# akashsengupta1997/indirect_learning_pose-shape

Measured on AMD Instinct MI355X. Metric: meshes/sec fwd+bwd (SMPL->48x48 31-part seg), higher is better.
Workload: dtype f32; 1 GPU; full decoder fwd+bwd (batch_smpl + projection + compute_mask + projects_to_seg), BASELINE configs[2]; meshes_per_gpu=128, global_batch=128, img_wh=48, vertex_sampling=1, verts=6890, params_per_mesh=86, launch=graph, steps_per_graph_launch=10, concurrent_chunks=1

## Files before the change

### include/smplraster.h

```cpp
#ifndef SMPLRASTER_H
#define SMPLRASTER_H

#include <stddef.h>
#include <stdint.h>

#ifdef __cplusplus
extern "C" {
#endif

#define SMPLR_ABI_VERSION 7
#define SMPLR_NJ 24
#define SMPLR_KPAD 220
#define SMPLR_CHUNK 8

#define SMPLR_EINVAL (-1)
#define SMPLR_EUNSUPPORTED (-2)

int smplr_abi_version(void);
const char *smplr_last_error(void);
int smplr_debug_device_ordinal(int fake_ordinal);
int smplr_debug_lds_attr_sets(void);
const char *smplr_build_id(void);


// ... 87 lines not shown
                           int16_t *arg, float *kernel_ms, void *stream);

int smplr_seg_raster_plan(int B, int W, int P, int K, int32_t *info, int32_t *tile_records);

int smplr_seg_bwd_nsplit(int B, int W);
size_t smplr_seg_bwd_workspace(int B, int W);
int smplr_seg_bwd(const float *dseg, const int16_t *arg, const float *rec,
                  int B, int VP, int W, int P, int K, float *dproj, void *workspace, int deterministic,
                  void *stream);

int smplr_seg_raster_ex(int B, int W, int P, int K, const void *workspace, const float *rec,
                        const int32_t *labels, const float *class_w, float gamma, float *seg, int16_t *arg,
                        float *loss, float *stats, float *vmax, void *stream);
int smplr_skin_vis_seg_fwd_ex(const float *v_posed, const float *lbs_top4, const float *A, const float *cam,
                              int x_stride, int B, int V, int W, int grid_wh, int ref_compat,
                              const int32_t *part_pos, const int32_t *part_off, int P, int K, void *workspace,
                              const int32_t *labels, const float *class_w, float gamma, float *verts, float *proj,
                              float *mask, float *seg, int16_t *arg, float *rec, int16_t *vslot, float *loss,
                              float *stats, float *vmax, void *stream);
int smplr_seg_loss_bwd(const float *dloss, const float *stats, const int16_t *arg, const float *rec, int B, int VP,
                       int W, int P, int K, float *dproj, void *workspace, int deterministic, void *stream);

int smplr_seg_confusion(const float *scores, const int32_t *pred, const int32_t *labels, long long npix, int C,
                        uint64_t *conf, uint8_t *pred_out, void *stream);
int smplr_seg_raster_ex_conf(int B, int W, int P, int K, const void *workspace, const float *rec,
                             const int32_t *labels, const float *class_w, float gamma, float *seg, int16_t *arg,
                             float *loss, float *stats, float *vmax, uint64_t *conf, void *stream);
int smplr_skin_vis_seg_fwd_ex_conf(const float *v_posed, const float *lbs_top4, const float *A, const float *cam,
                                   int x_stride, int B, int V, int W, int grid_wh, int ref_compat,
                                   const int32_t *part_pos, const int32_t *part_off, int P, int K, void *workspace,
                                   const int32_t *labels, const float *class_w, float gamma, float *verts, float *proj,
                                   float *mask, float *seg, int16_t *arg, float *rec, int16_t *vslot, float *loss,
                                   float *stats, float *vmax, uint64_t *conf, void *stream);

#define SMPLR_MESH_ORTHO 0
#define SMPLR_MESH_PERSPECTIVE 1
#define SMPLR_MESH_LAMBERT 0
#define SMPLR_MESH_VERTEX_COLOR 1
size_t smplr_mesh_vbuf_bytes(int B, int V);
int smplr_mesh_vertex(const float *verts, const float *cam, const float *trans, int B, int V, int mode, float scale,
                      int H, int W, float znear, float zfar, int shading, const int32_t *faces, int F,
                      const int32_t *vf_off, const int32_t *vf_face, int nnz, const float *light, int nlights,
                      const float *vcol, long long vcol_bstride, void *vbuf, void *stream);
int smplr_mesh_raster(const void *vbuf, const int32_t *faces, const uint8_t *face_part, int B, int V, int F, int H,
                      int W, int mode, const float *bg, int32_t *face, float *depth, uint8_t *part, uint8_t *alpha,
                      float *rgb, void *stream);

#define SMPLR_WARP_IMAGE_NEAREST 0
#define SMPLR_WARP_IMAGE_BILINEAR 1
#define SMPLR_WARP_LABEL 2
#define SMPLR_WARP_LABEL_BINARY 3
int smplr_affine_warp(const uint8_t *pool, int N, int Hs, int Ws, int C, const float *mat, const void *index,
                      int index_i64, int B, int H, int W, int mode, float rescale, void *out, void *stream);

#define SMPLR_RESIZE_IMAGE_BILINEAR 0
#define SMPLR_RESIZE_IMAGE_NEAREST 1
#define SMPLR_RESIZE_LABEL 2
#define SMPLR_RESIZE_LABEL_BINARY 3
#define SMPLR_RESIZE_PAD 1
#define SMPLR_RESIZE_SWAP_RB 2
#define SMPLR_RESIZE_QUANTIZE 4
#define SMPLR_RESIZE_PIL 8
int smplr_resize_pad(const uint8_t *data, long long data_bytes, const long long *desc, int N, int C, const void *index,
                     int index_i64, int B, int H, int W, int mode, int flags, float rescale, void *out, void *stream);

#define SMPLR_PE_NONE 0
// ... 120 lines not shown
```

### indirect_learning_pose-shape_amd/_lib.py

```python
from __future__ import annotations

import ctypes
import os
from ctypes import c_char_p, c_float, c_int, c_longlong, c_size_t, c_void_p

import torch

_HERE = os.path.dirname(os.path.abspath(__file__))
LIB_OVERRIDE = os.environ.get("SMPLR_LIB_PATH") or None
LIB_PATH = os.path.abspath(LIB_OVERRIDE) if LIB_OVERRIDE else os.path.join(_HERE, "libsmplraster_hip.so")

KPAD = 220
CHUNK = 8
ABI_VERSION = 7

P = c_void_p
I = c_int

SIGNATURES = {
    "smplr_abi_version": (c_int, []),
    "smplr_last_error": (c_char_p, []),
    "smplr_build_id": (c_char_p, []),
    "smplr_debug_device_ordinal": (c_int, [I]),
    "smplr_debug_lds_attr_sets": (c_int, []),
# ... 11 lines not shown
    "smplr_blend3_fwd": (c_int, [P, P, P, I, I, P, P]),
    "smplr_pose_blend3_fwd": (c_int, [P, I, I, I, P, P, P, P, P, I, P, P, P, P, P, P]),
    "smplr_blend3_bwd_workspace": (c_size_t, [I, I]),
    "smplr_blend3_bwd": (c_int, [P, P, I, I, P, P, P]),
    "smplr_skin_fwd": (c_int, [P, P, P, P, P, I, I, I, I, P, P, P]),
    "smplr_skin_bwd_workspace": (c_size_t, [I, I]),
    "smplr_skin_bwd": (c_int, [P, P, P, P, P, P, P, I, I, I, I, P, P, P, P, P]),
    "smplr_smpl_bwd_workspace": (c_size_t, [I, I]),
    "smplr_smpl_bwd": (c_int, [P, P, P, P, I, P, P, I, I, I, I, I, P, P, P, P, P, P, P, P, P, P, P, P, P]),
    "smplr_project_fwd": (c_int, [P, P, I, I, I, I, P, P]),
    "smplr_project_bwd": (c_int, [P, P, P, I, I, I, I, P, P, P]),
    "smplr_visibility": (c_int, [P, I, I, I, I, P, P]),
    "smplr_seg_workspace": (c_size_t, [I, I, I, I, I]),
    "smplr_seg_slots": (c_int, [I, I]),
    "smplr_seg_fwd": (c_int, [P, P, I, I, I, P, P, I, I, P, P, P, P, P, P]),
    "smplr_vis_seg_fwd": (c_int, [P, I, I, I, I, I, P, P, I, I, P, P, P, P, P, P, P]),
    "smplr_skin_vis_seg_fits": (c_int, [I, I, I]),
    "smplr_skin_vis_seg_fwd": (c_int, [P, P, P, P, I, I, I, I, I, I, P, P, I, I, P, P, P, P, P, P, P, P, P]),
    "smplr_seg_bin": (c_int, [P, P, I, I, I, I, I, P, P, I, I, P, P, P, P]),
    "smplr_seg_raster": (c_int, [I, I, I, I, P, P, P, P, P]),
    "smplr_seg_raster_timed": (c_int, [I, I, I, I, P, P, P, P, P, P]),
    "smplr_seg_raster_plan": (c_int, [I, I, I, I, P, P]),
    "smplr_seg_bwd_nsplit": (c_int, [I, I]),
    "smplr_seg_bwd_workspace": (c_size_t, [I, I]),
    "smplr_seg_bwd": (c_int, [P, P, P, I, I, I, I, I, P, P, I, P]),
    "smplr_seg_raster_ex": (c_int, [I, I, I, I, P, P, P, P, c_float, P, P, P, P, P, P]),
    "smplr_skin_vis_seg_fwd_ex": (c_int, [P, P, P, P, I, I, I, I, I, I, P, P, I, I, P, P, P, c_float, P, P, P, P, P, P,
                                          P, P, P, P, P]),
    "smplr_seg_loss_bwd": (c_int, [P, P, P, P, I, I, I, I, I, P, P, I, P]),
    "smplr_seg_confusion": (c_int, [P, P, P, c_longlong, I, P, P, P]),
    "smplr_seg_raster_ex_conf": (c_int, [I, I, I, I, P, P, P, P, c_float, P, P, P, P, P, P, P]),
    "smplr_skin_vis_seg_fwd_ex_conf": (c_int, [P, P, P, P, I, I, I, I, I, I, P, P, I, I, P, P, P, c_float, P, P, P, P, P,
                                               P, P, P, P, P, P, P]),
    "smplr_mesh_vbuf_bytes": (c_size_t, [I, I]),
    "smplr_mesh_vertex": (c_int, [P, P, P, I, I, I, c_float, I, I, c_float, c_float, I, P, I, P, P, I, P, I, P, c_longlong,
                                  P, P]),
    "smplr_mesh_raster": (c_int, [P, P, P, I, I, I, I, I, I, P, P, P, P, P, P, P]),
    "smplr_affine_warp": (c_int, [P, I, I, I, I, P, P, I, I, I, I, I, c_float, P, P]),
    "smplr_resize_pad": (c_int, [P, c_longlong, P, I, I, P, I, I, I, I, I, I, c_float, P, P]),
    "smplr_point_errors": (c_int, [P, P, I, I, I, I, P, P, P, P, P]),
    "smplr_mesh_measures": (c_int, [P, P, P, P, c_longlong, P, I, I, I, I, P, P, P, P, P, P, P, P]),
    "smplr_mesh_measures_bwd": (c_int, [P, P, P, P, I, P, P, c_longlong, P, P, P, P, P, P, P, I, I, I, I, P, P]),
    "smplr_seg_colour": (c_int, [P, P, I, I, I, I, P, I, I, P, I, I, I, P, P]),
    "smplr_scatter_points": (c_int, [P, P, P, I, P, I, I, I, I, c_float, I, I, I, I, P, P, P]),
    "smplr_fit_step": (c_int, [P, P, P, P, P, P, P, P, P, P, P, P, P, I, P, I, c_float, P, P, I, I, I, c_float, c_float, c_float,
                               c_float, c_float, I, I, P]),
    "smplr_prior_energy": (c_int, [P, I, I, I, P, P, P, P, P, P, I, I, P, P, P, P, P]),
    "smplr_fit_step_prior": (c_int, [P, P, P, P, P, P, P, P, P, P, P, P, P, I, P, I, c_float, P, P, I, I, I, c_float, c_float,
                                     c_float, c_float, c_float, I, I, I, P, P, P, P, P, P, I, I, P, P]),
    "smplr_silh_workspace": (c_size_t, [I, I, I]),
    "smplr_silh_fwd": (c_int, [P, I, I, I, P, P, P, P]),
    "smplr_silh_fwd_hint": (c_int, [P, P, I, I, I, P, P, P, P]),
    "smplr_silh_fwd_form": (c_int, [I, I]),
    "smplr_silh_bwd": (c_int, [P, P, P, P, I, I, I, P, I, P]),
    "smplr_silh_loss_fwd": (c_int, [P, P, P, c_float, I, I, P, P, P, P]),
    "smplr_silh_fwd_loss": (c_int, [P, P, P, P, c_float, I, I, I, P, P, P, P, P, P, P]),
    "smplr_silh_loss_bwd": (c_int, [P, P, P, P, P, I, I, I, P, I, P]),
    "smplr_focal_fwd": (c_int, [P, P, P, P, c_float, c_longlong, I, P, P, P]),
    "smplr_focal_bwd": (c_int, [P, P, P, P, c_float, P, c_longlong, I, P, P]),
    "smplr_prelu_fwd": (c_int, [P, P, c_longlong, I, I, P, P]),
    "smplr_prelu_bwd_workspace": (c_size_t, [c_longlong, I, I]),
    "smplr_prelu_bwd": (c_int, [P, P, P, c_longlong, I, I, P, P, P, P]),
    "smplr_bn_workspace": (c_size_t, [c_longlong, I, I]),
    "smplr_bn_fwd": (c_int, [P, P, P, P, c_longlong, I, I, c_float, c_float, P, P, P, P, P, P, P]),
    "smplr_bn_bwd": (c_int, [P, P, P, P, P, P, P, c_longlong, I, I, P, P, P, P, P, P]),
    "smplr_bn_res_fwd": (c_int, [P, P, P, P, P, P, c_longlong, I, I, c_float, c_float, P, P, P, P, P, P, P]),
# ... 116 lines not shown
```

### indirect_learning_pose-shape_amd/csrc/raster.hip

```cpp
#include <algorithm>
#include <tuple>
#include "raster_device.h"

namespace smplr {
#ifdef SMPLR_TL
constexpr int TL_RASTER_WG = 1152;
__device__ unsigned g_tl_raster[TL_RASTER_WG * 16 * 32];
#endif

constexpr int PLN = 128;
__host__ inline int raster2_shape(int B, int W, int K) {
  const long long nl = (long long)((W + 1) / 2) * W, blocks1 = (long long)B * ((nl + PLN - 1) / PLN);
  return (W <= 48 && K >= 6000 && blocks1 <= 900) ? 2 : 1;
}
constexpr int R2_STATIC = 1;
constexpr int R2_MAX = 11;

struct R2Block { int pl, ng; };
__host__ __device__ constexpr R2Block raster2_block(int shape) {
  return shape == 2 ? R2Block{64, 10} : shape == 3 ? R2Block{PLN, 4} : R2Block{PLN, 8};
}
__host__ __device__ constexpr int raster2_arena(int pl) { return pl == 64 ? 6144 : ARENA; }
__host__ __device__ constexpr int raster2_group_rows(int nrows) {
  return nrows <= 4 ? 5 : nrows <= 6 ? 7 : nrows <= 8 ? 9 : R2_MAX;
// ... 545 lines not shown
}

int smplr_seg_raster_ex_conf(int B, int W, int P, int K, const void *workspace, const float *rec, const int32_t *labels,
                             const float *class_w, float gamma, float *seg, int16_t *arg, float *loss, float *stats,
                             float *vmax, uint64_t *conf, void *stream) {
  return smplr::seg_raster_impl("smplr_seg_raster_ex", B, W, P, K, workspace, rec, seg, arg, stream,
                                smplr::LossOut{labels, class_w, gamma, loss, reinterpret_cast<float4 *>(stats), vmax},
                                nullptr, conf);
}

int smplr_skin_vis_seg_fwd_ex(const float *v_posed, const float *lbs_top4, const float *A, const float *cam,
                              int x_stride, int B, int V, int W, int grid_wh, int ref_compat, const int32_t *part_pos,
                              const int32_t *part_off, int P, int K, void *workspace, const int32_t *labels,
                              const float *class_w, float gamma, float *verts, float *proj, float *mask, float *seg,
                              int16_t *arg, float *rec, int16_t *vslot, float *loss, float *stats, float *vmax,
                              void *stream) {
  return smplr_skin_vis_seg_fwd_ex_conf(v_posed, lbs_top4, A, cam, x_stride, B, V, W, grid_wh, ref_compat, part_pos,
                                        part_off, P, K, workspace, labels, class_w, gamma, verts, proj, mask, seg, arg,
                                        rec, vslot, loss, stats, vmax, nullptr, stream);
}

int smplr_skin_vis_seg_fwd_ex_conf(const float *v_posed, const float *lbs_top4, const float *A, const float *cam,
                                   int x_stride, int B, int V, int W, int grid_wh, int ref_compat,
                                   const int32_t *part_pos, const int32_t *part_off, int P, int K, void *workspace,
                                   const int32_t *labels, const float *class_w, float gamma, float *verts, float *proj,
                                   float *mask, float *seg, int16_t *arg, float *rec, int16_t *vslot, float *loss,
                                   float *stats, float *vmax, uint64_t *conf, void *stream) {
  const smplr::SkinIn sk{v_posed, lbs_top4, A, cam, x_stride, verts, proj};
  return smplr::seg_fwd_impl("smplr_skin_vis_seg_fwd_ex", &sk, proj, mask, true, grid_wh, ref_compat, B, V, W, part_pos,
                             part_off, P, K, workspace, seg, arg, rec, vslot, stream,
                             smplr::LossOut{labels, class_w, gamma, loss, reinterpret_cast<float4 *>(stats), vmax}, conf);
}

}

#ifdef SMPLR_TL
SMPLR_TL_EXPORT(raster, smplr::g_tl_raster, smplr::TL_RASTER_WG * 16 * 32)
#endif
```

### indirect_learning_pose-shape_amd/csrc/seg_bin.hip

```cpp
#include "raster_common.h"
#include "skin_device.h"

namespace smplr {
constexpr int BIN_Q0 = 3;
constexpr float X_ZERO = 104.0f;
constexpr float M_LOCAL = 208.0f;
#ifdef SMPLR_TL
constexpr int TL_BIN_WG = 128;
__device__ unsigned g_tl_bin[TL_BIN_WG * (BIN_T / 64) * 32];
#endif

struct Slot {
  int cls;
  int pos, pix;
  float u, v, m, x;
};

__device__ __forceinline__ Slot classify(float u, float v, float m, int pos, int W) {
  Slot s;
  s.pos = pos;
  s.u = u;
  s.v = v;
  s.m = m;
  s.cls = 1;
// ... 267 lines not shown
      for (int q = 0; q < 31; ++q) rank += (__builtin_amdgcn_readlane(key, q) > key) ? 1 : 0;
      if (l < P) goffn[P + 2 + rank] = l;
    }
  }
  SMPLR_TL_STAMP(13);
  __syncthreads();
  SMPLR_TL_STAMP(14);
  {
    int p = p0;
    int run = gbase;
#pragma unroll
    for (int j = 0; j < IPT_MAX; ++j) {
      const int k = k0 + j;
      if (!(j < ipt && k < k1)) continue;
      while (k >= s_poff[p + 1]) ++p;
      const Slot s = sl[j];
      if (s.cls == 1) {
        const int slot = s_gpad[p] + (run - s_gstart[p]);
        Gn[slot] = make_float4(s.u, s.v, s.m * s.m, __int_as_float(s.pos));
        if (vslot) vsl[s.pos] = (short)slot;
        ++run;
      } else if (s.cls == 2) {
        const int dst = atomicAdd(&s_cnt[s.pix], 1);
        lrecn[dst] = make_uint2(__float_as_uint(s.x), (unsigned)p);
        Gn[s_gpad[P] + dst] = make_float4(s.u, s.v, s.m * s.m, __int_as_float(s.pos));
        if (vslot) vsl[s.pos] = (short)(s_gpad[P] + dst);
      }
    }
  }
  SMPLR_TL_STAMP(15);
  if (tid == 0) goffn[P + 1] = s_nonunit;
  if (tid == 0)
    Gn[S - 1] = make_float4(__int_as_float(s_gpad[P] + lstartn[npix]), __int_as_float(s_nonunit), __int_as_float(s_gpad[P]),
                            __int_as_float(-1));
  if (tid < P) {
    const int cnt = s_gstart[tid + 1] - s_gstart[tid];
    for (int i = s_gpad[tid] + cnt; i < s_gpad[tid + 1]; ++i)
      Gn[i] = make_float4(INFINITY, INFINITY, 1.0f, __int_as_float(-1));
  }
  SMPLR_TL_STAMP(16);
  SMPLR_TL_STAMP(17);
  SMPLR_TL_STAMP(18);
}

struct BinLds { size_t base, total; bool stage; };
static BinLds bin_lds(int VP, int W, int grid_wh ) {
  BinLds b;
  b.base = (size_t)((W * W + 1) & ~1) * sizeof(int);
  if (grid_wh > 0) b.base += (size_t)grid_wh * grid_wh * 8 + (size_t)((VP + 31) / 32) * 4;
  b.stage = b.base + (size_t)VP * 8 <= 150 * 1024;
  b.total = b.base + (b.stage ? (size_t)VP * 8 : 0);
  return b;
}

int seg_bin_impl(const char *fn, const float *proj, float *mask, bool fuse_vis, int grid_wh, int ref_compat, int B, int VP,
                 int W, const int32_t *part_pos, const int32_t *part_off, int P, int K, void *workspace, float *rec,
                 int16_t *vslot, void *stream, SkinIn sk) {
  SMPLR_REQUIRE(B >= 0 && VP > 0 && VP <= 32767 && W > 0 && W <= 160 && P >= 1 && P <= 31 && K > 0 && K <= BIN_T * IPT_MAX,
                "%s: bad sizes B=%d VP=%d W=%d (max 160) P=%d (max 31) K=%d", fn, B, VP, W, P, K);
  SMPLR_REQUIRE(!fuse_vis || (grid_wh > 0 && grid_wh <= 128), "%s: bad grid_wh=%d (max 128)", fn, grid_wh);
  if (B == 0) return 0;
  const bool skin = sk.v_posed != nullptr;
  SMPLR_REQUIRE((skin || (proj && mask)) && part_pos && part_off && workspace && rec, "%s: null pointer", fn);
  SMPLR_REQUIRE(!skin || (sk.top4 && sk.A && sk.cam && sk.x_stride >= 4 && sk.proj == proj && fuse_vis &&
                          VP <= 7 * BIN_T),
                "%s: the skinning form needs the sparse weights, A, camera rows, the fused mask and V <= %d",
                fn, 7 * BIN_T);
  hipStream_t st = as_stream(stream);
  const SegWs ws = seg_ws_layout(B, W, P, K);
  const int S = seg_slots(P, K);
  char *base = reinterpret_cast<char *>(workspace);
  float4 *G = reinterpret_cast<float4 *>(rec);
  int *goff = reinterpret_cast<int *>(base + ws.goff_off);
  int *lstart = reinterpret_cast<int *>(base + ws.lstart_off);
  uint2 *lrec = reinterpret_cast<uint2 *>(base + ws.lrec_off);
  const BinLds bl = bin_lds(VP, W, fuse_vis ? grid_wh : 0);
  SMPLR_REQUIRE(bl.base <= 150 * 1024, "%s: pixel counters + grid + flags need %zu B of LDS (max 153600)", fn, bl.base);
  const bool stage = bl.stage;
  const size_t lds = bl.total;
#define SMPLR_BIN_LAUNCH(VIS_, STAGE_, SKIN_)                                                                 \
  {                                                                                                           \
    int rc = lds_attr<&seg_bin_kernel<VIS_, STAGE_, SKIN_>>(lds);          \
    if (rc) return rc;                                                                                        \
    hipLaunchKernelGGL((seg_bin_kernel<VIS_, STAGE_, SKIN_>), dim3(B), dim3(BIN_T), lds, st, proj, mask,      \
                       part_pos, part_off, P, K, VP, W, S, G, goff, lstart, lrec, fuse_vis ? grid_wh : 1,     \
                       ref_compat, reinterpret_cast<short *>(vslot), sk);                                     \
  }
  SMPLR_REQUIRE(!skin || stage, "%s: the skinning form needs the staged (u, v) to fit LDS", fn);
  if (skin) SMPLR_BIN_LAUNCH(true, true, true)
  else if (fuse_vis && stage) SMPLR_BIN_LAUNCH(true, true, false)
  else if (fuse_vis) SMPLR_BIN_LAUNCH(true, false, false)
  else if (stage) SMPLR_BIN_LAUNCH(false, true, false)
  else SMPLR_BIN_LAUNCH(false, false, false)
#undef SMPLR_BIN_LAUNCH
  SMPLR_LAUNCH_CHECK(fn);
  return 0;
}
}

extern "C" {

int smplr_seg_slots(int P, int K) { return (P > 0 && K > 0) ? smplr::seg_slots(P, K) : 0; }

size_t smplr_seg_workspace(int B, int VP, int W, int P, int K) {
  if (B <= 0 || VP <= 0 || W <= 0 || P <= 0 || K <= 0) return 0;
  return smplr::seg_ws_layout(B, W, P, K).total;
}

int smplr_seg_bin(const float *proj, float *mask, int B, int VP, int W, int grid_wh, int ref_compat,
                  const int32_t *part_pos, const int32_t *part_off, int P, int K, void *workspace, float *rec,
                  int16_t *vslot, void *stream) {
  return smplr::seg_bin_impl("smplr_seg_bin", proj, mask, grid_wh > 0, grid_wh, ref_compat, B, VP, W, part_pos,
                             part_off, P, K, workspace, rec, vslot, stream);
}

int smplr_skin_vis_seg_fits(int V, int W, int grid_wh) {
  if (V <= 0 || V > 7 * smplr::BIN_T || W <= 0 || W > 160 || grid_wh <= 0 || grid_wh > 128) return 0;
  const smplr::BinLds b = smplr::bin_lds(V, W, grid_wh);
  return (b.base <= 150 * 1024 && b.stage) ? 1 : 0;
}

}
// ... 5 lines not shown
```

### indirect_learning_pose-shape_amd/csrc/skin_device.h

```cpp
#pragma once
#include "common.h"

namespace smplr {

typedef float f32x4 __attribute__((ext_vector_type(4)));

__device__ __forceinline__ void skin_T_sparse(const float4 *sAj, const float4 ww, const float4 jj, float T[12]) {
  const float w[4] = {ww.x, ww.y, ww.z, ww.w};
  const int jx[4] = {(int)jj.x, (int)jj.y, (int)jj.z, (int)jj.w};
#pragma unroll
  for (int e = 0; e < 12; ++e) T[e] = 0.0f;
#pragma unroll
  for (int k = 0; k < 4; ++k) {
    const float4 r0 = sAj[jx[k] * 3], r1 = sAj[jx[k] * 3 + 1], r2 = sAj[jx[k] * 3 + 2];
    const float wj = w[k];
    T[0] = fmaf(wj, r0.x, T[0]); T[1] = fmaf(wj, r0.y, T[1]); T[2] = fmaf(wj, r0.z, T[2]); T[3] = fmaf(wj, r0.w, T[3]);
    T[4] = fmaf(wj, r1.x, T[4]); T[5] = fmaf(wj, r1.y, T[5]); T[6] = fmaf(wj, r1.z, T[6]); T[7] = fmaf(wj, r1.w, T[7]);
    T[8] = fmaf(wj, r2.x, T[8]); T[9] = fmaf(wj, r2.y, T[9]); T[10] = fmaf(wj, r2.z, T[10]); T[11] = fmaf(wj, r2.w, T[11]);
  }
}
__device__ __forceinline__ void skin_apply(const float T[12], float p0, float p1, float p2, float &X, float &Y, float &Z) {
  X = T[0] * p0 + T[1] * p1 + T[2] * p2 + T[3];
  Y = T[4] * p0 + T[5] * p1 + T[6] * p2 + T[7];
  Z = T[8] * p0 + T[9] * p1 + T[10] * p2 + T[11];
}
__device__ __forceinline__ float project_u(float X, float c0, float c2) { return c2 + X * c0; }

struct SkinIn { const float *v_posed, *top4, *A, *cam; int x_stride; float *verts, *proj; };

inline int vp_count(int V, int vs) { return (V + vs - 1) / vs; }
struct SampledVertex {
  bool sampled; int vpi;
  __device__ __forceinline__ SampledVertex(int v, int vs) : sampled(vs <= 1 || v % vs == 0), vpi(vs <= 1 ? v : v / vs) {}
};

template <bool SPARSE> struct SkinWeights;
template <> struct SkinWeights<true> {
  static constexpr int N = 4;
  float4 ww, jj;
  __device__ __forceinline__ SkinWeights(const float *, const float *top4, int v) {
    const float4 *tp = reinterpret_cast<const float4 *>(top4 + (size_t)v * 8);
    ww = tp[0]; jj = tp[1];
  }
  __device__ __forceinline__ float weight(int k) const { return k == 0 ? ww.x : (k == 1 ? ww.y : (k == 2 ? ww.z : ww.w)); }
  __device__ __forceinline__ int joint(int k) const { return (int)(k == 0 ? jj.x : (k == 1 ? jj.y : (k == 2 ? jj.z : jj.w))); }
};
template <> struct SkinWeights<false> {
  static constexpr int N = 24;
  float w[24];
  __device__ __forceinline__ SkinWeights(const float *lbs, const float *, int v) {
    const float4 *wp = reinterpret_cast<const float4 *>(lbs + (size_t)v * 24);
#pragma unroll
    for (int q = 0; q < 6; ++q) {
      const float4 t = wp[q];
      w[4 * q] = t.x; w[4 * q + 1] = t.y; w[4 * q + 2] = t.z; w[4 * q + 3] = t.w;
    }
  }
  __device__ __forceinline__ float weight(int k) const { return w[k]; }
  __device__ __forceinline__ int joint(int k) const { return k; }
};

// ... 88 lines not shown
```

### indirect_learning_pose-shape_amd/ops.py

```python
from __future__ import annotations

import os
from dataclasses import dataclass
from typing import Optional

import numpy as np
import torch

from . import _lib
from ._lib import KPAD, CHUNK, check, on_device, ptr, require_cuda, stream
from .smpl_model import SMPLModelData, load_part_tables


@dataclass
class SMPLConstants:
    V: int
    v_template: torch.Tensor
    blend: torch.Tensor
    blend_t: torch.Tensor
    J_template: torch.Tensor
    J_dirs: torch.Tensor
    lbs_weights: torch.Tensor
    parents: torch.Tensor
    joint_regressor: Optional[torch.Tensor] = None
# ... 44 lines not shown
        dev = self.blend.device
        self.blend3_fwd = torch.empty(lib.smplr_blend3_fwd_bytes(N3), dtype=torch.uint8, device=dev)
        self.blend3_bwd = torch.empty(lib.smplr_blend3_bwd_bytes(N3), dtype=torch.uint8, device=dev)
        with torch.cuda.device(dev):
            check(lib.smplr_blend3_pack(ptr(self.blend), N3, ptr(self.blend3_fwd), ptr(self.blend3_bwd), stream()),
                  "smplr_blend3_pack")
        return self

    def as_list(self):
        e = lambda t, dt=torch.float32: t if t is not None else torch.empty(0, dtype=dt, device=self.v_template.device)
        return [self.J_template, self.J_dirs, self.parents, self.v_template, e(self.blend3_fwd, torch.uint8),
                e(self.blend3_bwd, torch.uint8), self.lbs_weights, e(self.lbs_top4), self.blend_t]

    def fp32_gemm(self):
        import dataclasses
        return dataclasses.replace(self, blend3_fwd=None, blend3_bwd=None)


def blend_gemm_mode() -> str:
    import os
    m = os.environ.get("SMPLR_BLEND_GEMM", "bf16x3").lower()
    if m not in ("bf16x3", "f32"):
        raise RuntimeError("SMPLR_BLEND_GEMM must be bf16x3 or f32, got %r" % m)
    return m


@dataclass
class PartTable:
    P: int
    K: int
    part_pos: torch.Tensor
    part_off: torch.Tensor
    VP: int


_part_tables = {}


def build_part_table(ids, off, vertex_sampling, num_verts, device) -> PartTable:
    vs = 1 if vertex_sampling in (None, 1) else int(vertex_sampling)
    P = len(off) - 1
    part_pos = (np.asarray(ids, np.int64) // vs).astype(np.int32)
    VP = (num_verts + vs - 1) // vs
    assert part_pos.min() >= 0 and part_pos.max() < VP and int(off[-1]) == len(part_pos)
    if len(np.unique(part_pos)) != len(part_pos):
        raise ValueError("part table lists a vertex position more than once (after // vertex_sampling): "
                         "each vertex may belong to at most one part")
    return PartTable(P=P, K=int(len(part_pos)),
                     part_pos=torch.as_tensor(part_pos).to(device),
                     part_off=torch.as_tensor(np.asarray(off, np.int32)).to(device), VP=VP)


def get_part_table(vertex_sampling, device, num_verts=6890) -> PartTable:
    key = (1 if vertex_sampling in (None, 1) else int(vertex_sampling), str(device), num_verts)
    if key not in _part_tables:
        ids, off = load_part_tables(vertex_sampling)
        _part_tables[key] = build_part_table(ids, off, vertex_sampling, num_verts, device)
    return _part_tables[key]


def _empty(shape, like, dtype=torch.float32):
    return torch.empty(shape, dtype=dtype, device=like.device)


def _workspace(nbytes, like):
    return torch.empty(max(int(nbytes), 4) // 4 + 1, dtype=torch.float32, device=like.device)


class PoseCoef:
    __slots__ = ("kmajor", "frag3", "B")

    def __init__(self, kmajor, frag3, B):
        self.kmajor, self.frag3, self.B = kmajor, frag3, B

    @property
    def device(self):
        return (self.kmajor if self.kmajor is not None else self.frag3).device

    @property
    def is_cuda(self):
        return self.device.type == "cuda"


# ... 128 lines not shown
    ws = _workspace(lib.smplr_seg_workspace(B, VP, W, pt.P, pt.K), proj)
    if out is not None:
        mask, seg, arg, rec = out
    else:
        mask = _empty((B, VP), proj)
        seg = _empty((B, W, W, pt.P + 1), proj)
        arg = _empty((B, W, W, 32), proj, torch.int16)
        rec = _empty((B, lib.smplr_seg_slots(pt.P, pt.K), 4), proj)
    check(lib.smplr_vis_seg_fwd(ptr(proj), B, VP, W, int(grid_wh), 1 if ref_compat else 0, ptr(pt.part_pos),
                                ptr(pt.part_off), pt.P, pt.K, ptr(ws), ptr(mask), ptr(seg), ptr(arg), ptr(rec),
                                ptr(vslot), stream()), "smplr_vis_seg_fwd")
    return mask, seg, arg, rec


@on_device
def _skin_vis_seg_fwd(v_posed, A, c: SMPLConstants, cam, W, pt: PartTable, grid_wh=64, ref_compat=True, out=None,
                      vslot=None):
    lib = _lib.load()
    B, V = v_posed.shape[0], c.V
    if c.lbs_top4 is None or pt.VP != V:
        raise RuntimeError("_skin_vis_seg_fwd needs <= 4 skinning weights per vertex and vertex_sampling = 1")
    if not lib.smplr_skin_vis_seg_fits(V, int(W), int(grid_wh)):
        raise RuntimeError("_skin_vis_seg_fwd: V=%d, W=%d, grid_wh=%d do not fit the binning workgroup's LDS "
                           "(smplr_skin_vis_seg_fits): call _skin_fwd and _vis_seg_fwd" % (V, W, grid_wh))
    ws = _workspace(lib.smplr_seg_workspace(B, V, W, pt.P, pt.K), v_posed)
    if out is not None:
        verts, proj, mask, seg, arg, rec = out
    else:
        verts, proj = _empty((B, V, 3), v_posed), _empty((B, V, 3), v_posed)
        mask = _empty((B, V), v_posed)
        seg = _empty((B, W, W, pt.P + 1), v_posed)
        arg = _empty((B, W, W, 32), v_posed, torch.int16)
        rec = _empty((B, lib.smplr_seg_slots(pt.P, pt.K), 4), v_posed)
    check(lib.smplr_skin_vis_seg_fwd(ptr(v_posed), ptr(c.lbs_top4), ptr(A), ptr(cam), cam.shape[1], B, V, W,
                                     int(grid_wh), 1 if ref_compat else 0, ptr(pt.part_pos), ptr(pt.part_off), pt.P,
                                     pt.K, ptr(ws), ptr(verts), ptr(proj), ptr(mask), ptr(seg), ptr(arg), ptr(rec),
                                     ptr(vslot), stream()), "smplr_skin_vis_seg_fwd")
    return verts, proj, mask, seg, arg, rec


@on_device
def _skin_vis_seg_fwd_ex(v_posed, A, c: SMPLConstants, cam, W, pt: PartTable, labels=None, class_w=None, gamma=0.0,
                         grid_wh=64, ref_compat=True, verts=None, proj=None, mask=None, seg=None, arg=None, rec=None,
                         vslot=None, loss=None, stats=None, vmax=None, conf=None):
    lib = _lib.load()
    B, V = v_posed.shape[0], c.V
    if c.lbs_top4 is None or pt.VP != V or not lib.smplr_skin_vis_seg_fits(V, int(W), int(grid_wh)):
        raise RuntimeError("_skin_vis_seg_fwd_ex: needs sparse skinning weights, vertex_sampling = 1 and sizes that fit "
                           "the binning workgroup's LDS (smplr_skin_vis_seg_fits)")
    ws = _workspace(lib.smplr_seg_workspace(B, V, W, pt.P, pt.K), v_posed)
    if arg is None:
        arg = _empty((B, W, W, 32), v_posed, torch.int16)
    if rec is None:
        rec = _empty((B, lib.smplr_seg_slots(pt.P, pt.K), 4), v_posed)
    if labels is not None:
        loss = _empty((B, W * W), v_posed) if loss is None else loss
        stats = _empty((B, W * W, 4), v_posed) if stats is None else stats
    else:
        loss = stats = None
    if conf is not None:
        check(lib.smplr_skin_vis_seg_fwd_ex_conf(ptr(v_posed), ptr(c.lbs_top4), ptr(A), ptr(cam), cam.shape[1], B, V, W,
                                                 int(grid_wh), 1 if ref_compat else 0, ptr(pt.part_pos),
                                                 ptr(pt.part_off), pt.P, pt.K, ptr(ws), ptr(labels), ptr(class_w),
                                                 float(gamma), ptr(verts), ptr(proj), ptr(mask), ptr(seg), ptr(arg),
                                                 ptr(rec), ptr(vslot), ptr(loss), ptr(stats), ptr(vmax), ptr(conf),
                                                 stream()), "smplr_skin_vis_seg_fwd_ex_conf")
        return loss, stats, arg, rec
    check(lib.smplr_skin_vis_seg_fwd_ex(ptr(v_posed), ptr(c.lbs_top4), ptr(A), ptr(cam), cam.shape[1], B, V, W,
                                        int(grid_wh), 1 if ref_compat else 0, ptr(pt.part_pos), ptr(pt.part_off),
                                        pt.P, pt.K, ptr(ws), ptr(labels), ptr(class_w), float(gamma), ptr(verts),
                                        ptr(proj), ptr(mask), ptr(seg), ptr(arg), ptr(rec), ptr(vslot), ptr(loss),
                                        ptr(stats), ptr(vmax), stream()), "smplr_skin_vis_seg_fwd_ex")
    return loss, stats, arg, rec


@on_device
def _seg_raster_ex(ws, rec, B, W, pt: PartTable, labels=None, class_w=None, gamma=0.0, seg=None, arg=None, loss=None,
                   stats=None, vmax=None, conf=None):
    lib = _lib.load()
    if arg is None:
        arg = _empty((B, W, W, 32), rec, torch.int16)
    if labels is not None:
        loss = _empty((B, W * W), rec) if loss is None else loss
        stats = _empty((B, W * W, 4), rec) if stats is None else stats
    else:
        loss = stats = None
    if conf is not None:
        check(lib.smplr_seg_raster_ex_conf(B, W, pt.P, pt.K, ptr(ws), ptr(rec), ptr(labels), ptr(class_w), float(gamma),
                                           ptr(seg), ptr(arg), ptr(loss), ptr(stats), ptr(vmax), ptr(conf), stream()),
              "smplr_seg_raster_ex_conf")
        return loss, stats, arg
    check(lib.smplr_seg_raster_ex(B, W, pt.P, pt.K, ptr(ws), ptr(rec), ptr(labels), ptr(class_w), float(gamma),
                                  ptr(seg), ptr(arg), ptr(loss), ptr(stats), ptr(vmax), stream()), "smplr_seg_raster_ex")
    return loss, stats, arg


def _seg_raster_loss(ws, rec, B, W, pt, labels, class_w, gamma, seg=None, arg=None, loss=None, stats=None):
    return _seg_raster_ex(ws, rec, B, W, pt, labels, class_w, gamma, seg=seg, arg=arg, loss=loss, stats=stats)


@on_device
def _seg_loss_bwd(dloss, stats, arg, rec, VP, W, pt: PartTable, merge=True, deterministic=False):
    lib = _lib.load()
    B = arg.shape[0]
    ws = _workspace(lib.smplr_seg_bwd_workspace(B, W), dloss)
# ... 697 lines not shown
        def run(lo, hi):
            dproj, seg_grad = None, None
            if dseg is not None:
                part, nsplit = _seg_bwd(dseg[lo:hi], arg[lo:hi], rec[lo:hi], VP, ctx.W, ctx.pt, merge=False,
                                        deterministic=ctx.det)
                seg_grad = (part, vslot[lo:hi], nsplit)
            elif dloss is not None:
                part, nsplit = _seg_loss_bwd(dloss[lo:hi], stats[lo:hi], arg[lo:hi], rec[lo:hi], VP, ctx.W, ctx.pt,
                                             merge=False, deterministic=ctx.det)
                seg_grad = (part, vslot[lo:hi], nsplit)
            if dsilh is not None:
                d2 = _silh_bwd(dsilh[lo:hi], silh[lo:hi], sarg[lo:hi], proj[lo:hi], ctx.Ws, ctx.det)
                dproj = d2 if dproj is None else dproj + d2
            elif dsloss is not None:
                dproj = _silh_loss_bwd(dsloss[lo:hi], sk[lo:hi], silh[lo:hi], sarg[lo:hi], proj[lo:hi], ctx.Ws, ctx.det)
            if dproj_in is not None:
                dproj = dproj_in[lo:hi] if dproj is None else dproj + dproj_in[lo:hi]
            dv = dverts[lo:hi] if dverts is not None else None
            if dv is None and dproj is None and seg_grad is None:
                dv = torch.zeros_like(v_posed[lo:hi])
            _smpl_bwd(x[lo:hi], ctx.num_cam, ctx.consts, Rs[lo:hi], J[lo:hi], A[lo:hi], v_posed[lo:hi], dv,
                      dproj, dJt[lo:hi] if dJt is not None else None, ctx.vs, out=dx[lo:hi], seg_grad=seg_grad)

        if x.shape[0] > 0:
            _run_chunks(ctx.bounds, x.device, run)
        return (dx,) + (None,) * 11


@on_device
def _skin_vis_seg_opt(v_posed, A, c, cam, W, pt, grid_wh, ref_compat, verts, proj, mask, seg, arg, rec, vslot):
    lib = _lib.load()
    B, V = v_posed.shape[0], c.V
    ws = _workspace(lib.smplr_seg_workspace(B, V, W, pt.P, pt.K), v_posed)
    check(lib.smplr_skin_vis_seg_fwd(ptr(v_posed), ptr(c.lbs_top4), ptr(A), ptr(cam), cam.shape[1], B, V, W,
                                     int(grid_wh), 1 if ref_compat else 0, ptr(pt.part_pos), ptr(pt.part_off), pt.P,
                                     pt.K, ptr(ws), ptr(verts), ptr(proj), ptr(mask), ptr(seg), ptr(arg), ptr(rec),
                                     ptr(vslot), stream()), "smplr_skin_vis_seg_fwd")
```

Before: 1.063 million meshes/s.

## Add vertex-ownership binning kernel using inverse part table and packed skinning rows

```diff
diff --git a/include/smplraster.h b/include/smplraster.h
--- a/include/smplraster.h
+++ b/include/smplraster.h
@@ -143,6 +143,14 @@
                                    const int32_t *labels, const float *class_w, float gamma, float *verts, float *proj,
                                    float *mask, float *seg, int16_t *arg, float *rec, int16_t *vslot, float *loss,
                                    float *stats, float *vmax, uint64_t *conf, void *stream);
+
+int smplr_skin_vis_seg_fwd_inv(const float *v_posed, const float *lbs_top4, const float *A, const float *cam,
+                               int x_stride, int B, int V, int W, int grid_wh, int ref_compat,
+                               const int32_t *part_pos, const int32_t *part_off, int P, int K, const int32_t *part_inv,
+                               const float *top4_packed, void *workspace, const int32_t *labels, const float *class_w,
+                               float gamma, float *verts, float *proj, float *mask, float *seg, int16_t *arg,
+                               float *rec, int16_t *vslot, float *loss, float *stats, float *vmax, uint64_t *conf,
+                               void *stream);
 
 #define SMPLR_MESH_ORTHO 0
 #define SMPLR_MESH_PERSPECTIVE 1
diff --git a/indirect_learning_pose-shape_amd/_lib.py b/indirect_learning_pose-shape_amd/_lib.py
--- a/indirect_learning_pose-shape_amd/_lib.py
+++ b/indirect_learning_pose-shape_amd/_lib.py
@@ -67,6 +67,8 @@
     "smplr_seg_raster_ex_conf": (c_int, [I, I, I, I, P, P, P, P, c_float, P, P, P, P, P, P, P]),
     "smplr_skin_vis_seg_fwd_ex_conf": (c_int, [P, P, P, P, I, I, I, I, I, I, P, P, I, I, P, P, P, c_float, P, P, P, P, P,
                                                P, P, P, P, P, P, P]),
+    "smplr_skin_vis_seg_fwd_inv": (c_int, [P, P, P, P, I, I, I, I, I, I, P, P, I, I, P, P, P, P, P, c_float, P, P, P, P,
+                                           P, P, P, P, P, P, P, P]),
     "smplr_mesh_vbuf_bytes": (c_size_t, [I, I]),
     "smplr_mesh_vertex": (c_int, [P, P, P, I, I, I, c_float, I, I, c_float, c_float, I, P, I, P, P, I, P, I, P, c_longlong,
                                   P, P]),
diff --git a/indirect_learning_pose-shape_amd/csrc/raster.hip b/indirect_learning_pose-shape_amd/csrc/raster.hip
--- a/indirect_learning_pose-shape_amd/csrc/raster.hip
+++ b/indirect_learning_pose-shape_amd/csrc/raster.hip
@@ -601,6 +601,20 @@
                              smplr::LossOut{labels, class_w, gamma, loss, reinterpret_cast<float4 *>(stats), vmax}, conf);
 }
 
+int smplr_skin_vis_seg_fwd_inv(const float *v_posed, const float *lbs_top4, const float *A, const float *cam,
+                                int x_stride, int B, int V, int W, int grid_wh, int ref_compat, const int32_t *part_pos,
+                                const int32_t *part_off, int P, int K, const int32_t *part_inv, const float *top4_packed,
+                                void *workspace, const int32_t *labels, const float *class_w, float gamma, float *verts,
+                                float *proj, float *mask, float *seg, int16_t *arg, float *rec, int16_t *vslot,
+                                float *loss, float *stats, float *vmax, uint64_t *conf, void *stream) {
+  SMPLR_REQUIRE((part_inv == nullptr) == (top4_packed == nullptr),
+                "smplr_skin_vis_seg_fwd_inv: part_inv and top4_packed come together");
+  const smplr::SkinIn sk{v_posed, lbs_top4, A, cam, x_stride, verts, proj, part_inv, top4_packed};
+  return smplr::seg_fwd_impl("smplr_skin_vis_seg_fwd_inv", &sk, proj, mask, true, grid_wh, ref_compat, B, V, W, part_pos,
+                             part_off, P, K, workspace, seg, arg, rec, vslot, stream,
+                             smplr::LossOut{labels, class_w, gamma, loss, reinterpret_cast<float4 *>(stats), vmax}, conf);
+}
+
 }
 
 #ifdef SMPLR_TL
diff --git a/indirect_learning_pose-shape_amd/csrc/seg_bin.hip b/indirect_learning_pose-shape_amd/csrc/seg_bin.hip
--- a/indirect_learning_pose-shape_amd/csrc/seg_bin.hip
+++ b/indirect_learning_pose-shape_amd/csrc/seg_bin.hip
@@ -323,6 +323,260 @@
   if (tid == 0) goffn[P + 1] = s_nonunit;
   if (tid == 0)
     Gn[S - 1] = make_float4(__int_as_float(s_gpad[P] + lstartn[npix]), __int_as_float(s_nonunit), __int_as_float(s_gpad[P]),
+                            __int_as_float(-1));
+  if (tid < P) {
+    const int cnt = s_gstart[tid + 1] - s_gstart[tid];
+    for (int i = s_gpad[tid] + cnt; i < s_gpad[tid + 1]; ++i)
+      Gn[i] = make_float4(INFINITY, INFINITY, 1.0f, __int_as_float(-1));
+  }
+  SMPLR_TL_STAMP(16);
+  SMPLR_TL_STAMP(17);
+  SMPLR_TL_STAMP(18);
+}
+
+constexpr int OWN_Q = 7;
+constexpr int OWN_FW = OWN_Q * BIN_T / 32;
+constexpr int INV_SLOT = 0xffff;
+static_assert(OWN_FW <= 4 * 64, "one wave scans the bitmap, four words per lane");
+
+__global__ __launch_bounds__(BIN_T) void seg_bin_own_kernel(float *__restrict__ mask, const int *__restrict__ part_off,
+                                                            int P, int K, int VP, int W, int S, float4 *__restrict__ G,
+                                                            int *__restrict__ goff, int *__restrict__ lstart,
+                                                            uint2 *__restrict__ lrec, int vgrid, int ref_compat,
+                                                            short *__restrict__ vslot, SkinIn sk) {
+  extern __shared__ __attribute__((aligned(16))) int s_cnt[];
+  __shared__ int s_poff[33], s_gstart[33], s_gpad[33], s_wave[BIN_T / 64], s_fbase[OWN_FW + 1];
+  __shared__ unsigned s_far[OWN_FW];
+  __shared__ int s_any_empty;
+  __shared__ float4 sAj[72];
+  const int n = blockIdx.x, tid = threadIdx.x, lane = tid & 63;
+  SMPLR_TL_WAVE(g_tl_bin, BIN_T / 64, n, TL_BIN_WG)
+  const int npix = W * W;
+  const int cells = vgrid * vgrid, words = (VP + 31) / 32;
+  unsigned long long *zbuf = reinterpret_cast<unsigned long long *>(s_cnt + ((npix + 1) & ~1));
+  unsigned int *vis = reinterpret_cast<unsigned int *>(zbuf + cells);
+
+  int sw[OWN_Q];
+#pragma unroll
+  for (int q = 0; q < OWN_Q; ++q) sw[q] = sk.inv[min(tid + q * BIN_T, VP - 1)];
+  const float4 aj = reinterpret_cast<const float4 *>(sk.A + (size_t)n * 288)[tid < 72 ? tid : 71];
+  const float *cm = sk.cam + (size_t)n * sk.x_stride;
+  const float c0 = cm[0], c1 = cm[1], c2 = cm[2], c3 = cm[3];
+  const float *vp = sk.v_posed + (size_t)n * VP * 3;
+  float vu[OWN_Q], vv[OWN_Q], vz[OWN_Q];
+  float4 tw[OWN_Q];
+  unsigned tj[OWN_Q];
+#pragma unroll
+  for (int q = 0; q < BIN_Q0; ++q) {
+    const int v = min(tid + q * BIN_T, VP - 1);
+    const float4 *tp = reinterpret_cast<const float4 *>(sk.top4p + (size_t)v * 8);
+    tw[q] = tp[0];
+    tj[q] = __float_as_uint(tp[1].x);
+    vu[q] = vp[v * 3 + 0];
+    vv[q] = vp[v * 3 + 1];
+    vz[q] = vp[v * 3 + 2];
+  }
+  if (tid <= P) s_poff[tid] = part_off[tid];
+  if (tid == 0) s_any_empty = 0;
+  for (int i = tid; i < npix; i += BIN_T) s_cnt[i] = 0;
+  for (int i = tid; i < cells; i += BIN_T) zbuf[i] = 0ull;
+  for (int i = tid; i < words; i += BIN_T) vis[i] = 0u;
+  if (tid < OWN_FW) s_far[tid] = 0u;
+  if (tid < 72) sAj[tid] = aj;
+  SMPLR_TL_STAMP(1);
+  __syncthreads();
+  SMPLR_TL_STAMP(2);
+#pragma unroll
+  for (int q = BIN_Q0; q < OWN_Q; ++q) {
+    const int v = min(tid + q * BIN_T, VP - 1);
+    const float4 *tp = reinterpret_cast<const float4 *>(sk.top4p + (size_t)v * 8);
+    tw[q] = tp[0];
+    tj[q] = __float_as_uint(tp[1].x);
+    vu[q] = vp[v * 3 + 0];
+    vv[q] = vp[v * 3 + 1];
+    vz[q] = vp[v * 3 + 2];
+  }
+  __builtin_amdgcn_sched_barrier(0);
+  {
+    float *vo = sk.verts + (size_t)n * VP * 3, *po = sk.proj + (size_t)n * VP * 3;
+    const float fG = (float)vgrid;
+#pragma unroll
+    for (int q = 0; q < OWN_Q; ++q) {
+      const int v = tid + q * BIN_T;
+      float T[12], X, Y, Z;
+      skin_T_sparse(sAj, tw[q], tj[q], T);
+      skin_apply(T, vu[q], vv[q], vz[q], X, Y, Z);
+      vu[q] = project_u(X, c0, c2);
+      vv[q] = project_u(Y, c1, c3);
+      if (v < VP) {
+        if (sk.verts) { SMPLR_OUT_STORE(&vo[v * 3 + 0], X); SMPLR_OUT_STORE(&vo[v * 3 + 1], Y); SMPLR_OUT_STORE(&vo[v * 3 + 2], Z); }
+        if (sk.proj) { SMPLR_OUT_STORE(&po[v * 3 + 0], vu[q]); SMPLR_OUT_STORE(&po[v * 3 + 1], vv[q]); SMPLR_OUT_STORE(&po[v * 3 + 2], Z); }
+        const float pu = rintf(vu[q]);
+        const float pv = rintf(vv[q]);
+        if (pu >= 0.0f && pu < fG && pv >= 0.0f && pv < fG) {
+          const int cell = (int)pv * vgrid + (int)pu;
+          const unsigned long long key = ((unsigned long long)orderable(Z) << 32) |
+                                         (unsigned long long)(0xFFFFFFFFu - (unsigned)v);
+          atomicMax(&zbuf[cell], key);
+        }
+      }
+      __builtin_amdgcn_sched_barrier(0);
+    }
+  }
+  SMPLR_TL_STAMP(3);
+  __syncthreads();
+  SMPLR_TL_STAMP(4);
+  {
+    int empty = 0;
+    for (int i = tid; i < cells; i += BIN_T) {
+      const unsigned long long key = zbuf[i];
+      if (key == 0ull) {
+        empty = 1;
+      } else {
+        const unsigned int v = 0xFFFFFFFFu - (unsigned int)(key & 0xFFFFFFFFull);
+        atomicOr(&vis[v >> 5], 1u << (v & 31));
+      }
+    }
+    if (empty) s_any_empty = 1;
+  }
+  SMPLR_TL_STAMP(5);
+  __syncthreads();
+  SMPLR_TL_STAMP(6);
+  SMPLR_TL_STAMP(7);
+  const bool vertex1 = s_any_empty && ref_compat && VP > 1;
+  float *mk = mask ? mask + (size_t)n * VP : nullptr;
+  short *vsl = vslot ? vslot + (size_t)n * VP : nullptr;
+  float4 *Gn = G + (size_t)n * S;
+  int *goffn = goff + (size_t)n * goff_stride(P);
+  int *lstartn = lstart + (size_t)n * (npix + 1);
+  uint2 *lrecn = lrec + (size_t)n * K;
+
+  int pk[OWN_Q];
+  float lx[OWN_Q];
+#pragma unroll
+  for (int q = 0; q < OWN_Q; ++q) {
+    const int v = tid + q * BIN_T, slot = min(sw[q] & INV_SLOT, K - 1);
+    const bool on = v < VP;
+    const int vb = on ? v : 0;
+    const float m = (((vis[vb >> 5] >> (vb & 31)) & 1u) || (vertex1 && v == 1)) ? 1.0f : 500.0f;
+    if (mk && on) SMPLR_OUT_STORE(&mk[v], m);
+    int cls = 0, pix = 0;
+    lx[q] = 0.f;
+    if (on && sw[q] >= 0) {
+      const Slot c = classify(vu[q], vv[q], m, v, W);
+      cls = c.cls;
+      pix = c.pix;
+      lx[q] = c.x;
+    }
+    if (cls == 1) atomicOr(&s_far[slot >> 5], 1u << (slot & 31));
+    if (cls == 2) atomicAdd(&s_cnt[pix], 1);
+    if (vsl && cls == 0 && on) vsl[v] = -1;
+    pk[q] = cls | (pix << 2);
+  }
+  SMPLR_TL_STAMP(8);
+  __syncthreads();
+  SMPLR_TL_STAMP(9);
+  const int ept = (npix + BIN_T - 1) / BIN_T;
+  const int e0 = tid * ept, e1 = min(npix, e0 + ept);
+  int loc = 0;
+  for (int e = e0; e < e1; ++e) loc += s_cnt[e];
+  int linc = loc;
+#pragma unroll
+  for (int o = 1; o < 64; o <<= 1) {
+    const int t = __shfl_up(linc, o, 64);
+    if (lane >= o) linc += t;
+  }
+  if (lane == 63) s_wave[tid >> 6] = linc;
+  if (tid >= BIN_T - 64) {
+    int c[4], inc = 0;
+#pragma unroll
+    for (int i = 0; i < 4; ++i) {
+      c[i] = 4 * lane + i < OWN_FW ? __popc(s_far[4 * lane + i]) : 0;
+      inc += c[i];
+    }
+    const int own = inc;
+#pragma unroll
+    for (int o = 1; o < 64; o <<= 1) {
+      const int t = __shfl_up(inc, o, 64);
+      if (lane >= o) inc += t;
+    }
+    int run = inc - own;
+#pragma unroll
+    for (int i = 0; i < 4; ++i) {
+      if (4 * lane + i < OWN_FW) s_fbase[4 * lane + i] = run;
+      run += c[i];
+    }
+    if (lane == 63) s_fbase[OWN_FW] = inc;
+  }
+  SMPLR_TL_STAMP(10);
+  SMPLR_TL_STAMP(11);
+  __syncthreads();
+  SMPLR_TL_STAMP(12);
+  int ltotal = 0;
+  {
+    int run = linc - loc;
+    for (int w = 0; w < BIN_T / 64; ++w) {
+      const int t = s_wave[w];
+      if (w < (tid >> 6)) run += t;
+      ltotal += t;
+    }
+    for (int e = e0; e < e1; ++e) {
+      const int c = s_cnt[e];
+      s_cnt[e] = run;
+      lstartn[e] = run;
+      run += c;
+    }
+    if (tid == 0) lstartn[npix] = ltotal;
+  }
+  if (tid < 128) {
+    const int l = tid & 63;
+    int gs = s_fbase[OWN_FW];
+    const int kk = s_poff[l <= P ? l : P];
+    if (l < P && kk < K) gs = s_fbase[kk >> 5] + __popc(s_far[kk >> 5] & ((1u << (kk & 31)) - 1u));
+    const int gnext = __shfl_down(gs, 1, 64);
+    const int cnt = (l < P) ? (gnext - gs + GP - 1) / GP * GP : 0;
+    if (tid < 64) {
+      int inc = cnt;
+#pragma unroll
+      for (int o = 1; o < 32; o <<= 1) {
+        const int t = __shfl_up(inc, o, 64);
+        if (tid >= o) inc += t;
+      }
+      if (tid <= P) {
+        s_gstart[tid] = gs;
+        s_gpad[tid] = inc - cnt;
+        goffn[tid] = inc - cnt;
+      }
+    } else {
+      const int key = l < P ? ((cnt << 5) | (31 - l)) : -1;
+      int rank = 0;
+#pragma unroll
+      for (int q = 0; q < 31; ++q) rank += (__builtin_amdgcn_readlane(key, q) > key) ? 1 : 0;
+      if (l < P) goffn[P + 2 + rank] = l;
+    }
+  }
+  SMPLR_TL_STAMP(13);
+  __syncthreads();
+  SMPLR_TL_STAMP(14);
+#pragma unroll
+  for (int q = 0; q < OWN_Q; ++q) {
+    const int v = tid + q * BIN_T, cls = pk[q] & 3, slot = min(sw[q] & INV_SLOT, K - 1), p = min((sw[q] >> 16) & 31, P - 1);
+    if (cls == 1) {
+      const int rank = s_fbase[slot >> 5] + __popc(s_far[slot >> 5] & ((1u << (slot & 31)) - 1u));
+      const int dst = s_gpad[p] + (rank - s_gstart[p]);
+      Gn[dst] = make_float4(vu[q], vv[q], 1.0f, __int_as_float(v));
+      if (vsl) vsl[v] = (short)dst;
+    } else if (cls == 2) {
+      const int dst = atomicAdd(&s_cnt[pk[q] >> 2], 1);
+      lrecn[dst] = make_uint2(__float_as_uint(lx[q]), (unsigned)p);
+      Gn[s_gpad[P] + dst] = make_float4(vu[q], vv[q], 500.0f * 500.0f, __int_as_float(v));
+      if (vsl) vsl[v] = (short)(s_gpad[P] + dst);
+    }
+  }
+  SMPLR_TL_STAMP(15);
+  if (tid == 0) goffn[P + 1] = 0;
+  if (tid == 0)
+    Gn[S - 1] = make_float4(__int_as_float(s_gpad[P] + ltotal), __int_as_float(0), __int_as_float(s_gpad[P]),
                             __int_as_float(-1));
   if (tid < P) {
     const int cnt = s_gstart[tid + 1] - s_gstart[tid];
@@ -378,7 +632,14 @@
                        ref_compat, reinterpret_cast<short *>(vslot), sk);                                     \
   }
   SMPLR_REQUIRE(!skin || stage, "%s: the skinning form needs the staged (u, v) to fit LDS", fn);
-  if (skin) SMPLR_BIN_LAUNCH(true, true, true)
+  const char *own_env = (skin && sk.inv) ? getenv("SMPLR_SEG_BIN_WALK") : nullptr;
+  if (skin && sk.inv && !(own_env && atoi(own_env) == 0)) {
+    SMPLR_REQUIRE(sk.top4p && K <= VP, "%s: the table by vertex comes with the packed skinning rows and K <= V", fn);
+    if (int rc = lds_launch<&seg_bin_own_kernel>(LdsLaunch(dim3(B), dim3(BIN_T), bl.base, st), mask, part_off, P, K, VP, W,
+                                                 S, G, goff, lstart, lrec, grid_wh, ref_compat,
+                                                 reinterpret_cast<short *>(vslot), sk))
+      return rc;
+  } else if (skin) SMPLR_BIN_LAUNCH(true, true, true)
   else if (fuse_vis && stage) SMPLR_BIN_LAUNCH(true, true, false)
   else if (fuse_vis) SMPLR_BIN_LAUNCH(true, false, false)
   else if (stage) SMPLR_BIN_LAUNCH(false, true, false)
diff --git a/indirect_learning_pose-shape_amd/csrc/skin_device.h b/indirect_learning_pose-shape_amd/csrc/skin_device.h
--- a/indirect_learning_pose-shape_amd/csrc/skin_device.h
+++ b/indirect_learning_pose-shape_amd/csrc/skin_device.h
@@ -5,9 +5,8 @@
 
 typedef float f32x4 __attribute__((ext_vector_type(4)));
 
-__device__ __forceinline__ void skin_T_sparse(const float4 *sAj, const float4 ww, const float4 jj, float T[12]) {
+__device__ __forceinline__ void skin_T_sparse(const float4 *sAj, const float4 ww, const int jx[4], float T[12]) {
   const float w[4] = {ww.x, ww.y, ww.z, ww.w};
-  const int jx[4] = {(int)jj.x, (int)jj.y, (int)jj.z, (int)jj.w};
 #pragma unroll
   for (int e = 0; e < 12; ++e) T[e] = 0.0f;
 #pragma unroll
@@ -19,6 +18,14 @@
     T[8] = fmaf(wj, r2.x, T[8]); T[9] = fmaf(wj, r2.y, T[9]); T[10] = fmaf(wj, r2.z, T[10]); T[11] = fmaf(wj, r2.w, T[11]);
   }
 }
+__device__ __forceinline__ void skin_T_sparse(const float4 *sAj, const float4 ww, const float4 jj, float T[12]) {
+  const int jx[4] = {(int)jj.x, (int)jj.y, (int)jj.z, (int)jj.w};
+  skin_T_sparse(sAj, ww, jx, T);
+}
+__device__ __forceinline__ void skin_T_sparse(const float4 *sAj, const float4 ww, const unsigned jp, float T[12]) {
+  const int jx[4] = {(int)(jp & 255u), (int)((jp >> 8) & 255u), (int)((jp >> 16) & 255u), (int)(jp >> 24)};
+  skin_T_sparse(sAj, ww, jx, T);
+}
 __device__ __forceinline__ void skin_apply(const float T[12], float p0, float p1, float p2, float &X, float &Y, float &Z) {
   X = T[0] * p0 + T[1] * p1 + T[2] * p2 + T[3];
   Y = T[4] * p0 + T[5] * p1 + T[6] * p2 + T[7];
@@ -26,7 +33,7 @@
 }
 __device__ __forceinline__ float project_u(float X, float c0, float c2) { return c2 + X * c0; }
 
-struct SkinIn { const float *v_posed, *top4, *A, *cam; int x_stride; float *verts, *proj; };
+struct SkinIn { const float *v_posed, *top4, *A, *cam; int x_stride; float *verts, *proj; const int *inv; const float *top4p; };
 
 inline int vp_count(int V, int vs) { return (V + vs - 1) / vs; }
 struct SampledVertex {
diff --git a/indirect_learning_pose-shape_amd/ops.py b/indirect_learning_pose-shape_amd/ops.py
--- a/indirect_learning_pose-shape_amd/ops.py
+++ b/indirect_learning_pose-shape_amd/ops.py
@@ -100,9 +100,59 @@
     part_pos: torch.Tensor
     part_off: torch.Tensor
     VP: int
+    inv: Optional[torch.Tensor] = None
+    top4_packed: Optional[tuple] = None
 
 
 _part_tables = {}
+WALK_MAX = 0x7fff
+
+
+def build_walk_table(part_pos, VP):
+    pos = np.asarray(part_pos, np.int64).reshape(-1)
+    if pos.size == 0 or VP > WALK_MAX or pos.min() < 0 or pos.max() >= VP:
+        return None
+    owned = np.zeros(VP, bool)
+    owned[pos] = True
+    if int(owned.sum()) != pos.size:
+        return None
+    walk = np.concatenate([pos, np.flatnonzero(~owned)])
+    assert walk.size == VP and np.array_equal(np.sort(walk), np.arange(VP))
+    return walk.astype(np.int32)
+
+
+def _part_inv(part_pos, off, VP):
+    walk = build_walk_table(part_pos, VP)
+    if walk is None:
+        return None
+    K = len(part_pos)
+    part = np.repeat(np.arange(len(off) - 1), np.diff(np.asarray(off, np.int64)))
+    inv = np.full(VP, -1, np.int32)
+    inv[walk[:K]] = np.arange(K) | (part << 16)
+    return inv
+
+
+def _inv_rows(pt: PartTable, c: SMPLConstants):
+    if pt.inv is None or c.lbs_top4 is None or pt.VP != c.V:
+        return None, None
+    if pt.top4_packed is None or pt.top4_packed[0] is not c.lbs_top4:
+        j = c.lbs_top4[:, 4:].to(torch.int32)
+        words = torch.zeros((c.V, 8), dtype=torch.int32, device=c.lbs_top4.device)
+        words[:, :4] = c.lbs_top4[:, :4].contiguous().view(torch.int32)
+        words[:, 4] = j[:, 0] | (j[:, 1] << 8) | (j[:, 2] << 16) | (j[:, 3] << 24)
+        pt.top4_packed = (c.lbs_top4, words)
+    return pt.inv, pt.top4_packed[1]
+
+
+def _skin_vis_seg_call(v_posed, A, c: SMPLConstants, cam, W, pt: PartTable, grid_wh, ref_compat, ws, labels=None,
+                       class_w=None, gamma=0.0, verts=None, proj=None, mask=None, seg=None, arg=None, rec=None, vslot=None,
+                       loss=None, stats=None, vmax=None, conf=None):
+    inv, top4p = _inv_rows(pt, c)
+    check(_lib.load().smplr_skin_vis_seg_fwd_inv(
+        ptr(v_posed), ptr(c.lbs_top4), ptr(A), ptr(cam), cam.shape[1], v_posed.shape[0], c.V, int(W), int(grid_wh),
+        1 if ref_compat else 0, ptr(pt.part_pos), ptr(pt.part_off), pt.P, pt.K, ptr(inv), ptr(top4p), ptr(ws), ptr(labels),
+        ptr(class_w), float(gamma), ptr(verts), ptr(proj), ptr(mask), ptr(seg), ptr(arg), ptr(rec), ptr(vslot), ptr(loss),
+        ptr(stats), ptr(vmax), ptr(conf), stream()), "smplr_skin_vis_seg_fwd_inv")
 
 
 def build_part_table(ids, off, vertex_sampling, num_verts, device) -> PartTable:
@@ -114,9 +164,11 @@
     if len(np.unique(part_pos)) != len(part_pos):
         raise ValueError("part table lists a vertex position more than once (after // vertex_sampling): "
                          "each vertex may belong to at most one part")
+    inv = _part_inv(part_pos, off, VP)
     return PartTable(P=P, K=int(len(part_pos)),
                      part_pos=torch.as_tensor(part_pos).to(device),
-                     part_off=torch.as_tensor(np.asarray(off, np.int32)).to(device), VP=VP)
+                     part_off=torch.as_tensor(np.asarray(off, np.int32)).to(device), VP=VP,
+                     inv=None if inv is None else torch.as_tensor(inv).to(device))
 
 
 def get_part_table(vertex_sampling, device, num_verts=6890) -> PartTable:
@@ -311,10 +363,8 @@
         seg = _empty((B, W, W, pt.P + 1), v_posed)
         arg = _empty((B, W, W, 32), v_posed, torch.int16)
         rec = _empty((B, lib.smplr_seg_slots(pt.P, pt.K), 4), v_posed)
-    check(lib.smplr_skin_vis_seg_fwd(ptr(v_posed), ptr(c.lbs_top4), ptr(A), ptr(cam), cam.shape[1], B, V, W,
-                                     int(grid_wh), 1 if ref_compat else 0, ptr(pt.part_pos), ptr(pt.part_off), pt.P,
-                                     pt.K, ptr(ws), ptr(verts), ptr(proj), ptr(mask), ptr(seg), ptr(arg), ptr(rec),
-                                     ptr(vslot), stream()), "smplr_skin_vis_seg_fwd")
+    _skin_vis_seg_call(v_posed, A, c, cam, W, pt, grid_wh, ref_compat, ws, verts=verts, proj=proj, mask=mask, seg=seg,
+                       arg=arg, rec=rec, vslot=vslot)
     return verts, proj, mask, seg, arg, rec
 
 
@@ -337,19 +387,8 @@
         stats = _empty((B, W * W, 4), v_posed) if stats is None else stats
     else:
         loss = stats = None
-    if conf is not None:
-        check(lib.smplr_skin_vis_seg_fwd_ex_conf(ptr(v_posed), ptr(c.lbs_top4), ptr(A), ptr(cam), cam.shape[1], B, V, W,
-                                                 int(grid_wh), 1 if ref_compat else 0, ptr(pt.part_pos),
-                                                 ptr(pt.part_off), pt.P, pt.K, ptr(ws), ptr(labels), ptr(class_w),
-                                                 float(gamma), ptr(verts), ptr(proj), ptr(mask), ptr(seg), ptr(arg),
-                                                 ptr(rec), ptr(vslot), ptr(loss), ptr(stats), ptr(vmax), ptr(conf),
-                                                 stream()), "smplr_skin_vis_seg_fwd_ex_conf")
-        return loss, stats, arg, rec
-    check(lib.smplr_skin_vis_seg_fwd_ex(ptr(v_posed), ptr(c.lbs_top4), ptr(A), ptr(cam), cam.shape[1], B, V, W,
-                                        int(grid_wh), 1 if ref_compat else 0, ptr(pt.part_pos), ptr(pt.part_off),
-                                        pt.P, pt.K, ptr(ws), ptr(labels), ptr(class_w), float(gamma), ptr(verts),
-                                        ptr(proj), ptr(mask), ptr(seg), ptr(arg), ptr(rec), ptr(vslot), ptr(loss),
-                                        ptr(stats), ptr(vmax), stream()), "smplr_skin_vis_seg_fwd_ex")
+    _skin_vis_seg_call(v_posed, A, c, cam, W, pt, grid_wh, ref_compat, ws, labels, class_w, gamma, verts, proj, mask, seg,
+                       arg, rec, vslot, loss, stats, vmax, conf)
     return loss, stats, arg, rec
 
 
@@ -1113,7 +1152,5 @@
     lib = _lib.load()
     B, V = v_posed.shape[0], c.V
     ws = _workspace(lib.smplr_seg_workspace(B, V, W, pt.P, pt.K), v_posed)
-    check(lib.smplr_skin_vis_seg_fwd(ptr(v_posed), ptr(c.lbs_top4), ptr(A), ptr(cam), cam.shape[1], B, V, W,
-                                     int(grid_wh), 1 if ref_compat else 0, ptr(pt.part_pos), ptr(pt.part_off), pt.P,
-                                     pt.K, ptr(ws), ptr(verts), ptr(proj), ptr(mask), ptr(seg), ptr(arg), ptr(rec),
-                                     ptr(vslot), stream()), "smplr_skin_vis_seg_fwd")
+    _skin_vis_seg_call(v_posed, A, c, cam, W, pt, grid_wh, ref_compat, ws, verts=verts, proj=proj, mask=mask, seg=seg,
+                       arg=arg, rec=rec, vslot=vslot)
```

Result: faster. 1.079 million meshes/s (median of 6 runs) (+1.5%).
